# zongh5a/MDF-Net

Hardware: AMD Instinct MI355X
Metric: views/sec at DTU 1600x1200x5-view x4-scale (higher is better)
Workload: dtype f32; 1 GPU; DTU eval 1600x1184 (1600x1200 cropped as load/dtueval.py:34), 5 views, 3 cost-volume stages + x2 refine = 4 output scales, hypotheses (48,24,8), batch 1 per rank, seeded random weights (pth/dtu_29.pth is not available offline); parallelism=views sharded over 1 rank(s), no collective

## Files before the change

### mdf-net_amd/csrc/wino2d.hip

```cpp
#include <cstdlib>
#include <type_traits>
#include "common.h"
#include "conv_lds_common.h"
#define W3_PINNED_TILES_32
#include "wino3d_acc.h"

namespace {

template <int I, int N, typename F>
__device__ __forceinline__ void static_for(F&& f) {
  if constexpr (I < N) {
    f(std::integral_constant<int, I>{});
    static_for<I + 1, N>(f);
  }
}

struct Wino2dParams {
  const float* x;
  const float* wpack;
  const float* alpha;
  const float* beta;
  const float* res;
  float* y;
  float res_scale;
  int B, H, W, relu;
  int tiles_h, tiles_w, n_tiles;
};

template <int CIN, int COUT>
struct W2 {
  static_assert(CIN % 16 == 0 && COUT % 16 == 0 && COUT <= 64 && CIN <= 128, "2-D Winograd form: Cin, Cout multiples of 16, Cout <= 64");
  static constexpr int PASSES = (CIN > 64) ? 2 : 1, CP = CIN / PASSES;
  static constexpr int NCH = CP / 16, NT = COUT / 16, NG = CP / 4;
  static constexpr int WN = (CP >= 64) ? 2 : 1, NTW = NT / WN, WM = 4 / WN;
  static_assert(NT % WN == 0 && NTW >= 1 && NTW <= 2, "cout tiles per wave");
  static constexpr int TH = 2 * WM, TWO = 32;
  static constexpr int PH = TH + 2, PW = TWO + 2;
  static constexpr int NPP = PH * PW;
  static constexpr int S = round_s(NPP, 4, 2);
  static constexpr int PLANE = CP * S;
  static constexpr int RING = 3;
  static constexpr int NPOS = NG * NPP;
  static constexpr int NFILL = (NPOS + 255) / 256;
  static constexpr int EPI_OFF = RING * PLANE;
  static constexpr int FRAG = 64 * 4;
  static constexpr int NSTEP = NCH * 16;
  static constexpr bool WL = ((size_t)(RING * PLANE + 128 + PASSES * NSTEP * NT * FRAG) * sizeof(float) <= 160 * 1024);
  static constexpr int W_OFF = EPI_OFF + 128;
  static constexpr size_t LDS_BYTES = (size_t)(RING * PLANE + 128 + (WL ? PASSES * NSTEP * NT * FRAG : 0)) * sizeof(float);
  static_assert(S > NPP, "a pad vector per group takes the fill's surplus lanes");
};

template <int CIN, bool S2D, bool SKIP, int PAD = 0>
struct W2Live {
  static constexpr int CM = CIN / 4, NSTEP = CIN;
  static constexpr bool all_odd(int ch, int bit) {
    for (int c = ch * 16; c < ch * 16 + 16; ++c)
      if (!(((c / CM) >> bit) & 1)) return false;
    return true;
  }
  static constexpr bool py1(int ch) { return S2D && SKIP && all_odd(ch, 1); }
  static constexpr bool px1(int ch) { return S2D && SKIP && all_odd(ch, 0); }
  static constexpr bool zero(int ch, int ab) { return (py1(ch) && (ab >> 2) == 3) || (px1(ch) && (ab & 3) == 3); }
  static constexpr bool kept(int ch, int ab) {
    if (!zero(ch, ab)) return false;
    int n = 0;
    for (int i = 0; i < ch * 16 + ab; ++i) n += zero(i / 16, i % 16) ? 1 : 0;
    return n < PAD;
  }
  static constexpr bool dead(int ch, int ab) { return zero(ch, ab) && !kept(ch, ab); }
  static constexpr bool kept_ok() {
    for (int i = 0; i < NSTEP; ++i)
      if (kept(i / 16, i % 16) && (i % 16 == 0 || zero(i / 16, i % 16 - 1))) return false;
    return true;
  }
  static constexpr bool need(int ch, int e) { return !(py1(ch) && (e >> 2) == 3) && !(px1(ch) && (e & 3) == 3); }
  static constexpr int count(int upto = NSTEP) {
    int n = 0;
    for (int i = 0; i < upto; ++i) n += dead(i / 16, i % 16) ? 0 : 1;
    return n;
  }
  static constexpr int nth(int j) {
    for (int i = 0; i < NSTEP; ++i)
      if (!dead(i / 16, i % 16) && j-- == 0) return i;
    return -1;
  }
  static constexpr bool chunk0_live() {
    for (int ab = 0; ab < 16; ++ab)
      if (dead(0, ab)) return false;
    return true;
  }
};

#ifndef MDF_W2_DIAG
#define MDF_W2_DIAG 0
#endif
#ifndef MDF_W2_HOLD_REL
#define MDF_W2_HOLD_REL 0
#endif
#ifndef MDF_W2_NA
#define MDF_W2_NA 4
#endif
#ifndef MDF_W2_WRITE_AB
#define MDF_W2_WRITE_AB 2
#endif

template <int CIN, int COUT, int NA, int WRITE_AB, bool S2D, bool SKIP = true, int PAD = 0>
__global__ __launch_bounds__(256, 1) void wino2d_kernel(const Wino2dParams p) {
  typedef W2<CIN, COUT> C;
  typedef W2Live<CIN, S2D, SKIP, PAD> LV;
  constexpr int NCH = C::NCH, NT = C::NT, S = C::S, PW = C::PW, NPP = C::NPP, NFILL = C::NFILL, NSTEP = C::NSTEP, PASSES = C::PASSES;
  constexpr int AH = NA - 1;
  constexpr int NL = LV::count();
  static_assert(PASSES * NSTEP == LV::NSTEP && (PASSES == 1 || S2D), "passes: the parity form only");
  static_assert(NA >= 2 && NL % NA == 0, "the fragment ring must close over a tile");
  static_assert(LV::chunk0_live(), "every accumulator tile's first step is in chunk 0 of pass 0 (mfma_fresh)");
  static_assert(LV::kept_ok(), "a kept zero step has a computed V[ab - 1]");
  extern __shared__ __attribute__((aligned(16))) float lds[];

  const int tid = threadIdx.x, lane = tid & 63;
  const int wave = __builtin_amdgcn_readfirstlane(tid >> 6);
  const int q = lane >> 4, n16 = lane & 15;
  const __amdgpu_buffer_rsrc_t wres = make_rsrc(p.wpack, (unsigned)(PASSES * NSTEP * NT * 64 * 4 * 4));
  const int wvoff = lane * 16;
  const int wm = wave / C::WN, wn = wave % C::WN;
  constexpr int NTW = C::NTW;
  const int lane_lds = (q * S + wm * 2 * PW + n16 * 2) * 4;

  if (tid < 128) {
    const int c = tid & 63;
    lds[C::EPI_OFF + tid] = (tid < 64) ? ((c < COUT && p.alpha) ? p.alpha[c] : 1.f) : ((c < COUT && p.beta) ? p.beta[c] : 0.f);
  }
  if constexpr (C::WL) {
    constexpr int NV = PASSES * NSTEP * NT * 64;
    for (int v = tid; v < NV; v += 256)
      *reinterpret_cast<float4*>(lds + C::W_OFF + v * 4) = *reinterpret_cast<const float4*>(p.wpack + (size_t)v * 4);
  }

  constexpr bool HOLD_REL = (NFILL <= 11) || (NTW == 1) || MDF_W2_HOLD_REL;
  constexpr int CM = S2D ? CIN / 4 : CIN;
  [[maybe_unused]] constexpr int GPP = CM / 4;
  static_assert(HOLD_REL ? PASSES == 1 : true, "held offsets are those of pass 0");
  auto rel_of = [&](int row, int col, int g, int pass) -> int {
    if constexpr (S2D) {
      const int gl = pass * C::NG + g, par = gl / GPP, c4 = gl - par * GPP;
      return (((2 * row + (par >> 1)) * (2 * p.W) + 2 * col + (par & 1)) * CM + c4 * 4) * 4;
    } else {
      return ((row * p.W + col) * CIN + g * 4) * 4;
    }
  };
  int f_lds[NFILL], f_rc[NFILL], f_rel[HOLD_REL ? NFILL : 1];
#pragma unroll
  for (int k = 0; k < NFILL; ++k) {
    const int idx = tid + k * 256;
    const int glo = idx & 3, r = idx >> 2;
    const int v = r % NPP, g = (r / NPP) * 4 + glo;
    const bool live = idx < C::NPOS;
    const int row = live ? v / PW : 0x40, col = v % PW;
    f_lds[k] = live ? (g * S + v) * 4 : NPP * 4;
    f_rc[k] = (row << 16) | (col << 8) | g;
    if constexpr (HOLD_REL) f_rel[k] = live ? rel_of(row, col, g, 0) : (int)0x80000000u;
  }

  const unsigned lb = mdf::xcd_remap(blockIdx.x, gridDim.x);
  const int t_begin = __builtin_amdgcn_readfirstlane((int)((unsigned long long)lb * (unsigned)p.n_tiles / gridDim.x));
  const int t_end = __builtin_amdgcn_readfirstlane((int)((unsigned long long)(lb + 1) * (unsigned)p.n_tiles / gridDim.x));
  if (t_begin >= t_end) return;

  float4 pf[NFILL];
  struct TileAt { int b, th, tw; };
  auto tile_at = [&](int t) -> TileAt {
    const int tw = t % p.tiles_w, rest = t / p.tiles_w;
    return TileAt{__builtin_amdgcn_readfirstlane(rest / p.tiles_h), __builtin_amdgcn_readfirstlane(rest % p.tiles_h), __builtin_amdgcn_readfirstlane(tw)};
  };
  auto tile_advance = [&](TileAt& c) {
    if (++c.tw == p.tiles_w) {
      c.tw = 0;
      if (++c.th == p.tiles_h) { c.th = 0; ++c.b; }
    }
  };
  auto issue_tile = [&](const TileAt& at, int pass, bool valid) {
    const int b = valid ? at.b : 0, h0 = (valid ? at.th : 0) * C::TH, w0 = (valid ? at.tw : 0) * C::TWO;
    const long long org = S2D ? ((long long)b * (2 * p.H) + 2 * (h0 - 1)) * (2 * p.W) + 2 * (w0 - 1)
                              : ((long long)b * p.H + (h0 - 1)) * p.W + (w0 - 1);
    const float* pz = p.x + org * CM;
    const unsigned long long pa = (unsigned long long)pz;
    const unsigned lo = (unsigned)__builtin_amdgcn_readfirstlane((int)(unsigned)pa), hi = (unsigned)__builtin_amdgcn_readfirstlane((int)(unsigned)(pa >> 32));
    const unsigned nrec = (!valid || (MDF_W2_DIAG & 1)) ? 0u : 0x7fffffffu;
    const __amdgpu_buffer_rsrc_t xr = make_rsrc((const void*)(((unsigned long long)hi << 32) | lo), nrec);
    const int r_lo = 1 - h0, r_hi = p.H + 1 - h0, c_lo = 1 - w0, c_hi = p.W + 1 - w0;
    if constexpr (HOLD_REL) {
      if (r_lo <= 0 && r_hi >= C::PH && c_lo <= 0 && c_hi >= C::PW) {
#pragma unroll
        for (int k = 0; k < NFILL; ++k) {
          const u32x4_t v = __builtin_amdgcn_raw_buffer_load_b128(xr, f_rel[k], 0, 0);
          pf[k] = make_float4(__uint_as_float(v.x), __uint_as_float(v.y), __uint_as_float(v.z), __uint_as_float(v.w));
        }
        return;
      }
    }
#pragma unroll
    for (int k = 0; k < NFILL; ++k) {
      const int row = f_rc[k] >> 16, col = (f_rc[k] >> 8) & 0xff;
      const bool ok = row >= r_lo && row < r_hi && col >= c_lo && col < c_hi;
      int rel;
      if constexpr (HOLD_REL) rel = f_rel[k];
      else rel = rel_of(row, col, f_rc[k] & 0xff, pass);
      const u32x4_t v = __builtin_amdgcn_raw_buffer_load_b128(xr, ok ? rel : (int)0x80000000u, 0, 0);
      pf[k] = make_float4(__uint_as_float(v.x), __uint_as_float(v.y), __uint_as_float(v.z), __uint_as_float(v.w));
    }
  };
  auto write_tile = [&](int slot) {
#pragma unroll
    for (int k = 0; k < NFILL; ++k) *reinterpret_cast<float4*>(lds + slot * C::PLANE + f_lds[k]) = pf[k];
  };

  f32x2_t V[16][2], Dn[16][2];
  auto read_elem = [&](int slot, int ch, int e) {
    const int i = e >> 2, j = e & 3;
    float t[4];
    lds_frag<4>(lds + slot * C::PLANE + lane_lds + ((ch * 4) * S + i * PW + j) * 4, t);
    Dn[e][0] = (f32x2_t){t[0], t[1]};
    Dn[e][1] = (f32x2_t){t[2], t[3]};
  };
  auto transform = [&](auto lcc) {
    constexpr int LC = decltype(lcc)::value;
    constexpr bool PY = LV::py1(LC), PX = LV::px1(LC);
#pragma unroll
    for (int j = 0; j < (PX ? 3 : 4); ++j)
#pragma unroll
      for (int c = 0; c < 2; ++c) {
        const f32x2_t d0 = Dn[j][c], d1 = Dn[4 + j][c], d2 = Dn[8 + j][c];
        Dn[j][c] = d0 - d2; Dn[4 + j][c] = d1 + d2; Dn[8 + j][c] = d2 - d1;
        if constexpr (!PY) { const f32x2_t d3 = Dn[12 + j][c]; Dn[12 + j][c] = d1 - d3; }
      }
#pragma unroll
    for (int a = 0; a < (PY ? 3 : 4); ++a)
#pragma unroll
      for (int c = 0; c < 2; ++c) {
        const f32x2_t e0 = Dn[a * 4][c], e1 = Dn[a * 4 + 1][c], e2 = Dn[a * 4 + 2][c];
        V[a * 4][c] = e0 - e2; V[a * 4 + 1][c] = e1 + e2; V[a * 4 + 2][c] = e2 - e1;
        if constexpr (!PX) { const f32x2_t e3 = Dn[a * 4 + 3][c]; V[a * 4 + 3][c] = e1 - e3; }
      }
#pragma unroll
    for (int e = 0; e < 16; ++e) {
      if ((PY && (e >> 2) == 3) || (PX && (e & 3) == 3)) continue;
#pragma unroll
      for (int c = 0; c < 2; ++c) asm volatile("" : "+v"(V[e][c]));
    }
  };

  float af[NA][NTW][4];
  auto load_a = [&](int i, int buf) {
#pragma unroll
    for (int ntl = 0; ntl < NTW; ++ntl) {
      if constexpr (C::WL) lds_frag<4>(lds + C::W_OFF + (i * NT + wn * NTW + ntl) * C::FRAG + lane * 4, af[buf][ntl]);
      else buf_load_to<4>(wres, wvoff, (i * NT + wn * NTW + ntl) * (64 * 4 * 4), af[buf][ntl]);
    }
  };

  auto epilogue = [&](const TileAt& at) {
    const int b = at.b, h0 = at.th * C::TH, w0 = at.tw * C::TWO;
    if (h0 + 2 * wm >= p.H) return;
    const float* epi_tab = lds + C::EPI_OFF;
    asm volatile("s_nop 15\n\ts_nop 15" ::: "memory");
    static_for<0, NTW>([&](auto ntc) {
      constexpr int nt = decltype(ntc)::value;
      const int c0 = (wn * NTW + nt) * 16 + 4 * q;
      float yv[2][2][4];
      static_for<0, 2>([&](auto k2c) {
        constexpr int k2 = decltype(k2c)::value;
        float m[16][2];
        static_for<0, 16>([&](auto abc) { AccTile<nt * 16 + decltype(abc)::value>::template read2<k2>(m[decltype(abc)::value]); });
        f32x2_t srow[2][4];
#pragma unroll
        for (int bb = 0; bb < 4; ++bb) {
          const f32x2_t m0 = {m[bb][0], m[bb][1]}, m1 = {m[4 + bb][0], m[4 + bb][1]};
          const f32x2_t m2 = {m[8 + bb][0], m[8 + bb][1]}, m3 = {m[12 + bb][0], m[12 + bb][1]};
          srow[0][bb] = m0 + m1 + m2;
          srow[1][bb] = m1 - m2 - m3;
        }
#pragma unroll
        for (int pr = 0; pr < 2; ++pr) {
          const f32x2_t y0 = srow[pr][0] + srow[pr][1] + srow[pr][2];
          const f32x2_t y1 = srow[pr][1] - srow[pr][2] - srow[pr][3];
          yv[pr][0][2 * k2] = y0[0]; yv[pr][0][2 * k2 + 1] = y0[1];
          yv[pr][1][2 * k2] = y1[0]; yv[pr][1][2 * k2 + 1] = y1[1];
        }
      });
      float al_l[4], be_l[4];
#pragma unroll
      for (int k = 0; k < 4; ++k) { al_l[k] = epi_tab[c0 + k]; be_l[k] = epi_tab[64 + c0 + k]; }
#pragma unroll
      for (int pr = 0; pr < 2; ++pr) {
        const int h = h0 + 2 * wm + pr;
        if (h >= p.H) continue;
        const size_t row_vox = ((size_t)b * p.H + h) * p.W;
#pragma unroll
        for (int rr = 0; rr < 2; ++rr) {
          const int ow = w0 + 2 * n16 + rr;
          if (ow >= p.W) continue;
          float ov[4];
#pragma unroll
          for (int k = 0; k < 4; ++k) {
            ov[k] = yv[pr][rr][k] * al_l[k] + be_l[k];
            if (p.relu) ov[k] = fmaxf(ov[k], 0.f);
          }
          const size_t oi = (row_vox + ow) * COUT + c0;
          if (p.res) {
            const float4 rv = *reinterpret_cast<const float4*>(p.res + oi);
            ov[0] = rv.x + ov[0] * p.res_scale; ov[1] = rv.y + ov[1] * p.res_scale;
            ov[2] = rv.z + ov[2] * p.res_scale; ov[3] = rv.w + ov[3] * p.res_scale;
          }
          if (!(MDF_W2_DIAG & 2) || ov[0] == 1234.5f) *reinterpret_cast<float4*>(p.y + oi) = make_float4(ov[0], ov[1], ov[2], ov[3]);
        }
      }
    });
  };

  auto step = [&](auto rc, auto pc, const TileAt& at, const TileAt& at_n, bool valid_n, bool has_next) {
    constexpr int R = decltype(rc)::value, P = decltype(pc)::value;
    constexpr int SLOT_N = (R + 1) % 3;
    constexpr int LC_NEXT = (P + 1 < PASSES) ? (P + 1) * NCH : 0;
    static_for<0, NSTEP>([&](auto ic) {
      constexpr int i = decltype(ic)::value;
      constexpr int ch = i / 16, ab = i % 16;
      constexpr int lc = P * NCH + ch, li = P * NSTEP + i;
      constexpr bool last_chunk = (ch == NCH - 1);
      constexpr bool live = !LV::dead(lc, ab);
      [[maybe_unused]] constexpr int j = LV::count(li);
      if constexpr (live) {
        constexpr int ahead = LV::nth((j + AH) % NL);
        if (!(MDF_W2_DIAG & 16)) load_a(ahead, (j + AH) % NA);
      }
      if constexpr (ch == 0 && ab == WRITE_AB) {
        if (has_next) {
          write_tile(SLOT_N);
          __syncthreads();
        }
      }
      if constexpr (ab > WRITE_AB && ab <= WRITE_AB + 8 && !(MDF_W2_DIAG & 32)) {
        constexpr int e0 = 2 * (ab - WRITE_AB - 1);
        constexpr int lcn = last_chunk ? LC_NEXT : lc + 1;
        static_for<0, 2>([&](auto kc) {
          constexpr int e = e0 + decltype(kc)::value;
          if constexpr (LV::need(lcn, e)) {
            if constexpr (!last_chunk) read_elem(R, ch + 1, e);
            else read_elem(SLOT_N, 0, e);
          }
        });
      }
      __builtin_amdgcn_sched_barrier(0);
      if constexpr (live) {
        static_for<0, NTW>([&](auto ntc) {
          constexpr int nt = decltype(ntc)::value;
          constexpr int T = nt * 16 + ab;
          constexpr int vb = LV::kept(lc, ab) ? ab - 1 : ab;
          if constexpr (lc == 0) AccTile<T>::mfma_fresh(af[j % NA][nt][0], V[vb][0][0]);
          else AccTile<T>::mfma(af[j % NA][nt][0], V[vb][0][0]);
          AccTile<T>::mfma(af[j % NA][nt][1], V[vb][0][1]);
          AccTile<T>::mfma(af[j % NA][nt][2], V[vb][1][0]);
          AccTile<T>::mfma(af[j % NA][nt][3], V[vb][1][1]);
        });
      }
      __builtin_amdgcn_sched_barrier(0);
      if constexpr (ab == 15 && !last_chunk) { if (!(MDF_W2_DIAG & 8)) transform(std::integral_constant<int, lc + 1>{}); }
    });
    issue_tile(at_n, P, valid_n);
    if (!(MDF_W2_DIAG & 8)) transform(std::integral_constant<int, LC_NEXT>{});
    if constexpr (P == PASSES - 1) { if (!(MDF_W2_DIAG & 4)) epilogue(at); }
  };

  int t = t_begin;
  const int t_last = t_end - 1;
  TileAt at = tile_at(t), at2 = at;
  issue_tile(at, 0, true);
  write_tile(0);
  __syncthreads();
  tile_advance(at2);
  if constexpr (PASSES == 1) {
    issue_tile(at2, 0, t < t_last);
    tile_advance(at2);
  } else {
    issue_tile(at, 1, true);
  }
#pragma unroll
  for (int e = 0; e < 16; ++e) read_elem(0, 0, e);
  transform(std::integral_constant<int, 0>{});
  static_for<0, AH>([&](auto ic) {
    constexpr int first = LV::nth(decltype(ic)::value);
    load_a(first, decltype(ic)::value % NA);
  });

#define W2_STEP(RR, PP)                                                                                                          \
  {                                                                                                                              \
    const bool more = t < t_last;                                                                                                \
    if constexpr (PASSES == 1) step(std::integral_constant<int, RR>{}, std::integral_constant<int, 0>{}, at, at2, t + 2 <= t_last, more); \
    else step(std::integral_constant<int, RR>{}, std::integral_constant<int, PP>{}, at, at2, more, (PP) == 0 || more);           \
    if constexpr ((PP) == PASSES - 1) {                                                                                          \
      if (!more) break;                                                                                                          \
      ++t; tile_advance(at); tile_advance(at2);                                                                                  \
    }                                                                                                                            \
  }
  if constexpr (PASSES == 1) {
    for (;;) {
      W2_STEP(0, 0)
      W2_STEP(1, 0)
      W2_STEP(2, 0)
    }
  } else {
    for (;;) {
      W2_STEP(0, 0)
      W2_STEP(1, 1)
      W2_STEP(2, 0)
      W2_STEP(0, 1)
      W2_STEP(1, 0)
      W2_STEP(2, 1)
    }
  }
#undef W2_STEP
}

template <int CIN, int COUT, bool S2D = false, bool SKIP = true, int NA = MDF_W2_NA, int PAD = 0>
int launch_wino2d(Wino2dParams& p, hipStream_t st) {
  typedef W2<CIN, COUT> C;
  constexpr int WRITE_AB = MDF_W2_WRITE_AB;
  p.tiles_h = (p.H + C::TH - 1) / C::TH;
  p.tiles_w = (p.W + C::TWO - 1) / C::TWO;
  const long long tiles = (long long)p.B * p.tiles_h * p.tiles_w;
  if (tiles >= (1ll << 31)) return MDF_EUNSUPPORTED;
  p.n_tiles = (int)tiles;
  constexpr auto kern = &wino2d_kernel<CIN, COUT, NA, WRITE_AB, S2D, S2D && SKIP, PAD>;
  if (int rc = mdf::ensure_dynamic_lds<kern>(C::LDS_BYTES)) return rc;
  long long grid = 256;
  grid = mdf::env_pos("MDF_WINO2D_GRID", grid);
  if (grid > tiles / 2) grid = tiles / 2;
  if (grid < 1) grid = 1;
  hipLaunchKernelGGL(kern, dim3((unsigned)grid), dim3(256), C::LDS_BYTES, st, p);
  return mdf::check_launch("wino2d_kernel");
}

}

int mdf_wino2d_dispatch(const float* x, const float* wpack_wino, const float* alpha, const float* beta, const float* res, float res_scale,
                        float* y, int B, int H, int W, int Cin, int Cout, int relu, void* stream) {
  Wino2dParams p{};
  p.x = x; p.wpack = wpack_wino; p.alpha = alpha; p.beta = beta; p.res = res; p.res_scale = res_scale; p.y = y;
  p.B = B; p.H = H; p.W = W; p.relu = relu;
  if ((long long)B * H * W * Cin * 4 >= (1ll << 31)) return MDF_EUNSUPPORTED;
  if (Cin == 16 && Cout == 16 && getenv("MDF_WINO2D_16")) return launch_wino2d<16, 16>(p, (hipStream_t)stream);
  if (Cin == 32 && Cout == 32) return launch_wino2d<32, 32>(p, (hipStream_t)stream);
  if (Cin == 64 && Cout == 64) return launch_wino2d<64, 64>(p, (hipStream_t)stream);
  return MDF_EUNSUPPORTED;
}

int mdf_wino2d_s2d_dispatch(const float* x, const float* wpack_k5w, const float* alpha, const float* beta, float* y, int B, int Ho, int Wo,
                            int Cin_mem, int Cout, int relu, void* stream) {
  Wino2dParams p{};
  p.x = x; p.wpack = wpack_k5w; p.alpha = alpha; p.beta = beta; p.res = nullptr; p.res_scale = 0.f; p.y = y;
  p.B = B; p.H = Ho; p.W = Wo; p.relu = relu;
  if ((long long)B * Ho * Wo * 4 * Cin_mem * 4 >= (1ll << 31)) return MDF_EUNSUPPORTED;
  const bool skip = mdf::env_flag("MDF_WINO2D_SKIP", true);
  hipStream_t st = (hipStream_t)stream;
  if (Cin_mem == 32 && Cout == 64) return skip ? launch_wino2d<128, 64, true, true, 4, 2>(p, st) : launch_wino2d<128, 64, true, false>(p, st);
  if (Cin_mem == 16 && Cout == 32) return skip ? launch_wino2d<64, 32, true, true, 7, 0>(p, st) : launch_wino2d<64, 32, true, false>(p, st);
  if (Cin_mem == 8 && Cout == 16) return launch_wino2d<32, 16, true, false>(p, st);
  return MDF_EUNSUPPORTED;
}
```

Before: 308.1 views/s.

## Cover ragged right edge of 2-D Winograd conv with narrow tall strip tiles

When the image width leaves a small remainder past the last full 32-wide tile column, the kernel now handles that remainder with 16x8 strip tiles instead of a full 8x32 tile that is mostly padding. The tile loop is wrapped in a templated run lambda, instantiated once for ordinary tiles and once for strips, and each block processes its ordinary range then its strip range. This cuts wasted MFMA and fill work on the mostly-empty edge tiles. The cost is a second code instantiation, which raises code size and register pressure, plus an extra barrier between the two phases. Strips can be turned off with an environment variable.

```diff
diff --git a/mdf-net_amd/csrc/wino2d.hip b/mdf-net_amd/csrc/wino2d.hip
--- a/mdf-net_amd/csrc/wino2d.hip
+++ b/mdf-net_amd/csrc/wino2d.hip
@@ -24,7 +24,10 @@
   float* y;
   float res_scale;
   int B, H, W, relu;
-  int tiles_h, tiles_w, n_tiles;
+  int tiles_h, tiles_w;
+  int strips_h;
+  int n_ord;
+  int n_tiles;
 };
 
 template <int CIN, int COUT>
@@ -37,6 +40,9 @@
   static constexpr int TH = 2 * WM, TWO = 32;
   static constexpr int PH = TH + 2, PW = TWO + 2;
   static constexpr int NPP = PH * PW;
+  static constexpr bool STRIPS = (WM == 2);
+  static constexpr int STH = 16, STW = 8, SPH = STH + 2, SPW = STW + 2;
+  static_assert(!STRIPS || (SPH * SPW <= NPP && STH == 8 * WM && TWO % STW == 0), "strip tiles: the patch fits the plane, 4 row pairs x 4 column pairs per wave");
   static constexpr int S = round_s(NPP, 4, 2);
   static constexpr int PLANE = CP * S;
   static constexpr int RING = 3;
@@ -109,7 +115,7 @@
 __global__ __launch_bounds__(256, 1) void wino2d_kernel(const Wino2dParams p) {
   typedef W2<CIN, COUT> C;
   typedef W2Live<CIN, S2D, SKIP, PAD> LV;
-  constexpr int NCH = C::NCH, NT = C::NT, S = C::S, PW = C::PW, NPP = C::NPP, NFILL = C::NFILL, NSTEP = C::NSTEP, PASSES = C::PASSES;
+  constexpr int NCH = C::NCH, NT = C::NT, S = C::S, NSTEP = C::NSTEP, PASSES = C::PASSES;
   constexpr int AH = NA - 1;
   constexpr int NL = LV::count();
   static_assert(PASSES * NSTEP == LV::NSTEP && (PASSES == 1 || S2D), "passes: the parity form only");
@@ -120,12 +126,10 @@
 
   const int tid = threadIdx.x, lane = tid & 63;
   const int wave = __builtin_amdgcn_readfirstlane(tid >> 6);
-  const int q = lane >> 4, n16 = lane & 15;
   const __amdgpu_buffer_rsrc_t wres = make_rsrc(p.wpack, (unsigned)(PASSES * NSTEP * NT * 64 * 4 * 4));
   const int wvoff = lane * 16;
   const int wm = wave / C::WN, wn = wave % C::WN;
   constexpr int NTW = C::NTW;
-  const int lane_lds = (q * S + wm * 2 * PW + n16 * 2) * 4;
 
   if (tid < 128) {
     const int c = tid & 63;
@@ -137,288 +141,322 @@
       *reinterpret_cast<float4*>(lds + C::W_OFF + v * 4) = *reinterpret_cast<const float4*>(p.wpack + (size_t)v * 4);
   }
 
-  constexpr bool HOLD_REL = (NFILL <= 11) || (NTW == 1) || MDF_W2_HOLD_REL;
-  constexpr int CM = S2D ? CIN / 4 : CIN;
-  [[maybe_unused]] constexpr int GPP = CM / 4;
-  static_assert(HOLD_REL ? PASSES == 1 : true, "held offsets are those of pass 0");
-  auto rel_of = [&](int row, int col, int g, int pass) -> int {
-    if constexpr (S2D) {
-      const int gl = pass * C::NG + g, par = gl / GPP, c4 = gl - par * GPP;
-      return (((2 * row + (par >> 1)) * (2 * p.W) + 2 * col + (par & 1)) * CM + c4 * 4) * 4;
-    } else {
-      return ((row * p.W + col) * CIN + g * 4) * 4;
-    }
-  };
-  int f_lds[NFILL], f_rc[NFILL], f_rel[HOLD_REL ? NFILL : 1];
-#pragma unroll
-  for (int k = 0; k < NFILL; ++k) {
-    const int idx = tid + k * 256;
-    const int glo = idx & 3, r = idx >> 2;
-    const int v = r % NPP, g = (r / NPP) * 4 + glo;
-    const bool live = idx < C::NPOS;
-    const int row = live ? v / PW : 0x40, col = v % PW;
-    f_lds[k] = live ? (g * S + v) * 4 : NPP * 4;
-    f_rc[k] = (row << 16) | (col << 8) | g;
-    if constexpr (HOLD_REL) f_rel[k] = live ? rel_of(row, col, g, 0) : (int)0x80000000u;
-  }
-
   const unsigned lb = mdf::xcd_remap(blockIdx.x, gridDim.x);
   const int t_begin = __builtin_amdgcn_readfirstlane((int)((unsigned long long)lb * (unsigned)p.n_tiles / gridDim.x));
   const int t_end = __builtin_amdgcn_readfirstlane((int)((unsigned long long)(lb + 1) * (unsigned)p.n_tiles / gridDim.x));
   if (t_begin >= t_end) return;
 
-  float4 pf[NFILL];
-  struct TileAt { int b, th, tw; };
-  auto tile_at = [&](int t) -> TileAt {
-    const int tw = t % p.tiles_w, rest = t / p.tiles_w;
-    return TileAt{__builtin_amdgcn_readfirstlane(rest / p.tiles_h), __builtin_amdgcn_readfirstlane(rest % p.tiles_h), __builtin_amdgcn_readfirstlane(tw)};
-  };
-  auto tile_advance = [&](TileAt& c) {
-    if (++c.tw == p.tiles_w) {
-      c.tw = 0;
-      if (++c.th == p.tiles_h) { c.th = 0; ++c.b; }
+  auto run = [&](auto kindc, const int t_b, const int t_e, [[maybe_unused]] const int n_ord, [[maybe_unused]] const int strips_h) {
+    constexpr bool STRIP = decltype(kindc)::value == 1;
+    constexpr int TH = STRIP ? C::STH : C::TH, PH = STRIP ? C::SPH : C::PH, PW = STRIP ? C::SPW : C::PW;
+    constexpr int NPP = PH * PW, NPOS = C::NG * NPP, NFILL = (NPOS + 255) / 256;
+    int tid_l = tid;
+    asm volatile("" : "+v"(tid_l));
+    const int q = (tid_l & 63) >> 4, n16 = tid_l & 15;
+    const int rp = STRIP ? 4 * wm + (n16 & 3) : wm, cp = STRIP ? (n16 >> 2) : n16;
+    const int lane_lds = (q * S + rp * 2 * PW + cp * 2) * 4;
+
+    constexpr bool HOLD_REL = (C::NFILL <= 11) || (NTW == 1) || MDF_W2_HOLD_REL;
+    constexpr int CM = S2D ? CIN / 4 : CIN;
+    [[maybe_unused]] constexpr int GPP = CM / 4;
+    static_assert(HOLD_REL ? PASSES == 1 : true, "held offsets are those of pass 0");
+    auto rel_of = [&](int row, int col, int g, int pass) -> int {
+      if constexpr (S2D) {
+        const int gl = pass * C::NG + g, par = gl / GPP, c4 = gl - par * GPP;
+        return (((2 * row + (par >> 1)) * (2 * p.W) + 2 * col + (par & 1)) * CM + c4 * 4) * 4;
+      } else {
+        return ((row * p.W + col) * CIN + g * 4) * 4;
+      }
+    };
+    int f_lds[NFILL], f_rc[NFILL], f_rel[HOLD_REL ? NFILL : 1];
+#pragma unroll
+    for (int k = 0; k < NFILL; ++k) {
+      const int idx = tid_l + k * 256;
+      const int glo = idx & 3, r = idx >> 2;
+      const int v = r % NPP, g = (r / NPP) * 4 + glo;
+      const bool live = idx < NPOS;
+      const int row = live ? v / PW : 0x40, col = v % PW;
+      f_lds[k] = live ? (g * S + v) * 4 : C::NPP * 4;
+      f_rc[k] = (row << 16) | (col << 8) | g;
+      if constexpr (HOLD_REL) f_rel[k] = live ? rel_of(row, col, g, 0) : (int)0x80000000u;
     }
-  };
-  auto issue_tile = [&](const TileAt& at, int pass, bool valid) {
-    const int b = valid ? at.b : 0, h0 = (valid ? at.th : 0) * C::TH, w0 = (valid ? at.tw : 0) * C::TWO;
-    const long long org = S2D ? ((long long)b * (2 * p.H) + 2 * (h0 - 1)) * (2 * p.W) + 2 * (w0 - 1)
-                              : ((long long)b * p.H + (h0 - 1)) * p.W + (w0 - 1);
-    const float* pz = p.x + org * CM;
-    const unsigned long long pa = (unsigned long long)pz;
-    const unsigned lo = (unsigned)__builtin_amdgcn_readfirstlane((int)(unsigned)pa), hi = (unsigned)__builtin_amdgcn_readfirstlane((int)(unsigned)(pa >> 32));
-    const unsigned nrec = (!valid || (MDF_W2_DIAG & 1)) ? 0u : 0x7fffffffu;
-    const __amdgpu_buffer_rsrc_t xr = make_rsrc((const void*)(((unsigned long long)hi << 32) | lo), nrec);
-    const int r_lo = 1 - h0, r_hi = p.H + 1 - h0, c_lo = 1 - w0, c_hi = p.W + 1 - w0;
-    if constexpr (HOLD_REL) {
-      if (r_lo <= 0 && r_hi >= C::PH && c_lo <= 0 && c_hi >= C::PW) {
-#pragma unroll
-        for (int k = 0; k < NFILL; ++k) {
-          const u32x4_t v = __builtin_amdgcn_raw_buffer_load_b128(xr, f_rel[k], 0, 0);
-          pf[k] = make_float4(__uint_as_float(v.x), __uint_as_float(v.y), __uint_as_float(v.z), __uint_as_float(v.w));
-        }
-        return;
-      }
-    }
-#pragma unroll
-    for (int k = 0; k < NFILL; ++k) {
-      const int row = f_rc[k] >> 16, col = (f_rc[k] >> 8) & 0xff;
-      const bool ok = row >= r_lo && row < r_hi && col >= c_lo && col < c_hi;
-      int rel;
-      if constexpr (HOLD_REL) rel = f_rel[k];
-      else rel = rel_of(row, col, f_rc[k] & 0xff, pass);
-      const u32x4_t v = __builtin_amdgcn_raw_buffer_load_b128(xr, ok ? rel : (int)0x80000000u, 0, 0);
-      pf[k] = make_float4(__uint_as_float(v.x), __uint_as_float(v.y), __uint_as_float(v.z), __uint_as_float(v.w));
-    }
-  };
-  auto write_tile = [&](int slot) {
-#pragma unroll
-    for (int k = 0; k < NFILL; ++k) *reinterpret_cast<float4*>(lds + slot * C::PLANE + f_lds[k]) = pf[k];
-  };
-
-  f32x2_t V[16][2], Dn[16][2];
-  auto read_elem = [&](int slot, int ch, int e) {
-    const int i = e >> 2, j = e & 3;
-    float t[4];
-    lds_frag<4>(lds + slot * C::PLANE + lane_lds + ((ch * 4) * S + i * PW + j) * 4, t);
-    Dn[e][0] = (f32x2_t){t[0], t[1]};
-    Dn[e][1] = (f32x2_t){t[2], t[3]};
-  };
-  auto transform = [&](auto lcc) {
-    constexpr int LC = decltype(lcc)::value;
-    constexpr bool PY = LV::py1(LC), PX = LV::px1(LC);
-#pragma unroll
-    for (int j = 0; j < (PX ? 3 : 4); ++j)
-#pragma unroll
-      for (int c = 0; c < 2; ++c) {
-        const f32x2_t d0 = Dn[j][c], d1 = Dn[4 + j][c], d2 = Dn[8 + j][c];
-        Dn[j][c] = d0 - d2; Dn[4 + j][c] = d1 + d2; Dn[8 + j][c] = d2 - d1;
-        if constexpr (!PY) { const f32x2_t d3 = Dn[12 + j][c]; Dn[12 + j][c] = d1 - d3; }
-      }
-#pragma unroll
-    for (int a = 0; a < (PY ? 3 : 4); ++a)
-#pragma unroll
-      for (int c = 0; c < 2; ++c) {
-        const f32x2_t e0 = Dn[a * 4][c], e1 = Dn[a * 4 + 1][c], e2 = Dn[a * 4 + 2][c];
-        V[a * 4][c] = e0 - e2; V[a * 4 + 1][c] = e1 + e2; V[a * 4 + 2][c] = e2 - e1;
-        if constexpr (!PX) { const f32x2_t e3 = Dn[a * 4 + 3][c]; V[a * 4 + 3][c] = e1 - e3; }
-      }
-#pragma unroll
-    for (int e = 0; e < 16; ++e) {
-      if ((PY && (e >> 2) == 3) || (PX && (e & 3) == 3)) continue;
-#pragma unroll
-      for (int c = 0; c < 2; ++c) asm volatile("" : "+v"(V[e][c]));
-    }
-  };
-
-  float af[NA][NTW][4];
-  auto load_a = [&](int i, int buf) {
-#pragma unroll
-    for (int ntl = 0; ntl < NTW; ++ntl) {
-      if constexpr (C::WL) lds_frag<4>(lds + C::W_OFF + (i * NT + wn * NTW + ntl) * C::FRAG + lane * 4, af[buf][ntl]);
-      else buf_load_to<4>(wres, wvoff, (i * NT + wn * NTW + ntl) * (64 * 4 * 4), af[buf][ntl]);
-    }
-  };
-
-  auto epilogue = [&](const TileAt& at) {
-    const int b = at.b, h0 = at.th * C::TH, w0 = at.tw * C::TWO;
-    if (h0 + 2 * wm >= p.H) return;
-    const float* epi_tab = lds + C::EPI_OFF;
-    asm volatile("s_nop 15\n\ts_nop 15" ::: "memory");
-    static_for<0, NTW>([&](auto ntc) {
-      constexpr int nt = decltype(ntc)::value;
-      const int c0 = (wn * NTW + nt) * 16 + 4 * q;
-      float yv[2][2][4];
-      static_for<0, 2>([&](auto k2c) {
-        constexpr int k2 = decltype(k2c)::value;
-        float m[16][2];
-        static_for<0, 16>([&](auto abc) { AccTile<nt * 16 + decltype(abc)::value>::template read2<k2>(m[decltype(abc)::value]); });
-        f32x2_t srow[2][4];
-#pragma unroll
-        for (int bb = 0; bb < 4; ++bb) {
-          const f32x2_t m0 = {m[bb][0], m[bb][1]}, m1 = {m[4 + bb][0], m[4 + bb][1]};
-          const f32x2_t m2 = {m[8 + bb][0], m[8 + bb][1]}, m3 = {m[12 + bb][0], m[12 + bb][1]};
-          srow[0][bb] = m0 + m1 + m2;
-          srow[1][bb] = m1 - m2 - m3;
-        }
-#pragma unroll
-        for (int pr = 0; pr < 2; ++pr) {
-          const f32x2_t y0 = srow[pr][0] + srow[pr][1] + srow[pr][2];
-          const f32x2_t y1 = srow[pr][1] - srow[pr][2] - srow[pr][3];
-          yv[pr][0][2 * k2] = y0[0]; yv[pr][0][2 * k2 + 1] = y0[1];
-          yv[pr][1][2 * k2] = y1[0]; yv[pr][1][2 * k2 + 1] = y1[1];
-        }
-      });
-      float al_l[4], be_l[4];
-#pragma unroll
-      for (int k = 0; k < 4; ++k) { al_l[k] = epi_tab[c0 + k]; be_l[k] = epi_tab[64 + c0 + k]; }
-#pragma unroll
-      for (int pr = 0; pr < 2; ++pr) {
-        const int h = h0 + 2 * wm + pr;
-        if (h >= p.H) continue;
-        const size_t row_vox = ((size_t)b * p.H + h) * p.W;
-#pragma unroll
-        for (int rr = 0; rr < 2; ++rr) {
-          const int ow = w0 + 2 * n16 + rr;
-          if (ow >= p.W) continue;
-          float ov[4];
-#pragma unroll
-          for (int k = 0; k < 4; ++k) {
-            ov[k] = yv[pr][rr][k] * al_l[k] + be_l[k];
-            if (p.relu) ov[k] = fmaxf(ov[k], 0.f);
+
+    float4 pf[NFILL];
+    struct TileAt { int b, th, tw; };
+    auto tile_at = [&](int t) -> TileAt {
+      if constexpr (STRIP) {
+        const int sl = t - n_ord;
+        return TileAt{__builtin_amdgcn_readfirstlane(sl / strips_h), __builtin_amdgcn_readfirstlane(sl % strips_h), p.tiles_w};
+      } else {
+        const int tw = t % p.tiles_w, rest = t / p.tiles_w;
+        return TileAt{__builtin_amdgcn_readfirstlane(rest / p.tiles_h), __builtin_amdgcn_readfirstlane(rest % p.tiles_h), __builtin_amdgcn_readfirstlane(tw)};
+      }
+    };
+    auto tile_advance = [&](TileAt& c) {
+      if constexpr (STRIP) {
+        if (++c.th == strips_h) { c.th = 0; ++c.b; }
+      } else {
+        if (++c.tw == p.tiles_w) {
+          c.tw = 0;
+          if (++c.th == p.tiles_h) { c.th = 0; ++c.b; }
+        }
+      }
+    };
+    auto issue_tile = [&](const TileAt& at, int pass, bool valid) {
+      const int b = valid ? at.b : 0, h0 = (valid ? at.th : 0) * TH, w0 = (valid ? at.tw : 0) * C::TWO;
+      const long long org = S2D ? ((long long)b * (2 * p.H) + 2 * (h0 - 1)) * (2 * p.W) + 2 * (w0 - 1)
+                                : ((long long)b * p.H + (h0 - 1)) * p.W + (w0 - 1);
+      const float* pz = p.x + org * CM;
+      const unsigned long long pa = (unsigned long long)pz;
+      const unsigned lo = (unsigned)__builtin_amdgcn_readfirstlane((int)(unsigned)pa), hi = (unsigned)__builtin_amdgcn_readfirstlane((int)(unsigned)(pa >> 32));
+      const unsigned nrec = (!valid || (MDF_W2_DIAG & 1)) ? 0u : 0x7fffffffu;
+      const __amdgpu_buffer_rsrc_t xr = make_rsrc((const void*)(((unsigned long long)hi << 32) | lo), nrec);
+      const int r_lo = 1 - h0, r_hi = p.H + 1 - h0, c_lo = 1 - w0, c_hi = p.W + 1 - w0;
+      if constexpr (HOLD_REL && !STRIP) {
+        if (r_lo <= 0 && r_hi >= PH && c_lo <= 0 && c_hi >= PW) {
+#pragma unroll
+          for (int k = 0; k < NFILL; ++k) {
+            const u32x4_t v = __builtin_amdgcn_raw_buffer_load_b128(xr, f_rel[k], 0, 0);
+            pf[k] = make_float4(__uint_as_float(v.x), __uint_as_float(v.y), __uint_as_float(v.z), __uint_as_float(v.w));
           }
-          const size_t oi = (row_vox + ow) * COUT + c0;
-          if (p.res) {
-            const float4 rv = *reinterpret_cast<const float4*>(p.res + oi);
-            ov[0] = rv.x + ov[0] * p.res_scale; ov[1] = rv.y + ov[1] * p.res_scale;
-            ov[2] = rv.z + ov[2] * p.res_scale; ov[3] = rv.w + ov[3] * p.res_scale;
+          return;
+        }
+      }
+#pragma unroll
+      for (int k = 0; k < NFILL; ++k) {
+        const int row = f_rc[k] >> 16, col = (f_rc[k] >> 8) & 0xff;
+        const bool ok = row >= r_lo && row < r_hi && col >= c_lo && col < c_hi;
+        int rel;
+        if constexpr (HOLD_REL) rel = f_rel[k];
+        else rel = rel_of(row, col, f_rc[k] & 0xff, pass);
+        const u32x4_t v = __builtin_amdgcn_raw_buffer_load_b128(xr, ok ? rel : (int)0x80000000u, 0, 0);
+        pf[k] = make_float4(__uint_as_float(v.x), __uint_as_float(v.y), __uint_as_float(v.z), __uint_as_float(v.w));
+      }
+    };
+    auto write_tile = [&](int slot) {
+#pragma unroll
+      for (int k = 0; k < NFILL; ++k) *reinterpret_cast<float4*>(lds + slot * C::PLANE + f_lds[k]) = pf[k];
+    };
+
+    f32x2_t V[16][2], Dn[16][2];
+    auto read_elem = [&](int slot, int ch, int e) {
+      const int i = e >> 2, j = e & 3;
+      float t[4];
+      lds_frag<4>(lds + slot * C::PLANE + lane_lds + ((ch * 4) * S + i * PW + j) * 4, t);
+      Dn[e][0] = (f32x2_t){t[0], t[1]};
+      Dn[e][1] = (f32x2_t){t[2], t[3]};
+    };
+    auto transform = [&](auto lcc) {
+      constexpr int LC = decltype(lcc)::value;
+      constexpr bool PY = LV::py1(LC), PX = LV::px1(LC);
+#pragma unroll
+      for (int j = 0; j < (PX ? 3 : 4); ++j)
+#pragma unroll
+        for (int c = 0; c < 2; ++c) {
+          const f32x2_t d0 = Dn[j][c], d1 = Dn[4 + j][c], d2 = Dn[8 + j][c];
+          Dn[j][c] = d0 - d2; Dn[4 + j][c] = d1 + d2; Dn[8 + j][c] = d2 - d1;
+          if constexpr (!PY) { const f32x2_t d3 = Dn[12 + j][c]; Dn[12 + j][c] = d1 - d3; }
+        }
+#pragma unroll
+      for (int a = 0; a < (PY ? 3 : 4); ++a)
+#pragma unroll
+        for (int c = 0; c < 2; ++c) {
+          const f32x2_t e0 = Dn[a * 4][c], e1 = Dn[a * 4 + 1][c], e2 = Dn[a * 4 + 2][c];
+          V[a * 4][c] = e0 - e2; V[a * 4 + 1][c] = e1 + e2; V[a * 4 + 2][c] = e2 - e1;
+          if constexpr (!PX) { const f32x2_t e3 = Dn[a * 4 + 3][c]; V[a * 4 + 3][c] = e1 - e3; }
+        }
+#pragma unroll
+      for (int e = 0; e < 16; ++e) {
+        if ((PY && (e >> 2) == 3) || (PX && (e & 3) == 3)) continue;
+#pragma unroll
+        for (int c = 0; c < 2; ++c) asm volatile("" : "+v"(V[e][c]));
+      }
+    };
+
+    float af[NA][NTW][4];
+    auto load_a = [&](int i, int buf) {
+#pragma unroll
+      for (int ntl = 0; ntl < NTW; ++ntl) {
+        if constexpr (C::WL) lds_frag<4>(lds + C::W_OFF + (i * NT + wn * NTW + ntl) * C::FRAG + lane * 4, af[buf][ntl]);
+        else buf_load_to<4>(wres, wvoff, (i * NT + wn * NTW + ntl) * (64 * 4 * 4), af[buf][ntl]);
+      }
+    };
+
+    auto epilogue = [&](const TileAt& at) {
+      const int b = at.b, h0 = at.th * TH, w0 = at.tw * C::TWO;
+      if (h0 + 2 * (STRIP ? 4 * wm : wm) >= p.H) return;
+      const float* epi_tab = lds + C::EPI_OFF;
+      asm volatile("s_nop 15\n\ts_nop 15" ::: "memory");
+      static_for<0, NTW>([&](auto ntc) {
+        constexpr int nt = decltype(ntc)::value;
+        const int c0 = (wn * NTW + nt) * 16 + 4 * q;
+        float yv[2][2][4];
+        static_for<0, 2>([&](auto k2c) {
+          constexpr int k2 = decltype(k2c)::value;
+          float m[16][2];
+          static_for<0, 16>([&](auto abc) { AccTile<nt * 16 + decltype(abc)::value>::template read2<k2>(m[decltype(abc)::value]); });
+          f32x2_t srow[2][4];
+#pragma unroll
+          for (int bb = 0; bb < 4; ++bb) {
+            const f32x2_t m0 = {m[bb][0], m[bb][1]}, m1 = {m[4 + bb][0], m[4 + bb][1]};
+            const f32x2_t m2 = {m[8 + bb][0], m[8 + bb][1]}, m3 = {m[12 + bb][0], m[12 + bb][1]};
+            srow[0][bb] = m0 + m1 + m2;
+            srow[1][bb] = m1 - m2 - m3;
           }
-          if (!(MDF_W2_DIAG & 2) || ov[0] == 1234.5f) *reinterpret_cast<float4*>(p.y + oi) = make_float4(ov[0], ov[1], ov[2], ov[3]);
-        }
-      }
-    });
-  };
-
-  auto step = [&](auto rc, auto pc, const TileAt& at, const TileAt& at_n, bool valid_n, bool has_next) {
-    constexpr int R = decltype(rc)::value, P = decltype(pc)::value;
-    constexpr int SLOT_N = (R + 1) % 3;
-    constexpr int LC_NEXT = (P + 1 < PASSES) ? (P + 1) * NCH : 0;
-    static_for<0, NSTEP>([&](auto ic) {
-      constexpr int i = decltype(ic)::value;
-      constexpr int ch = i / 16, ab = i % 16;
-      constexpr int lc = P * NCH + ch, li = P * NSTEP + i;
-      constexpr bool last_chunk = (ch == NCH - 1);
-      constexpr bool live = !LV::dead(lc, ab);
-      [[maybe_unused]] constexpr int j = LV::count(li);
-      if constexpr (live) {
-        constexpr int ahead = LV::nth((j + AH) % NL);
-        if (!(MDF_W2_DIAG & 16)) load_a(ahead, (j + AH) % NA);
-      }
-      if constexpr (ch == 0 && ab == WRITE_AB) {
-        if (has_next) {
-          write_tile(SLOT_N);
-          __syncthreads();
-        }
-      }
-      if constexpr (ab > WRITE_AB && ab <= WRITE_AB + 8 && !(MDF_W2_DIAG & 32)) {
-        constexpr int e0 = 2 * (ab - WRITE_AB - 1);
-        constexpr int lcn = last_chunk ? LC_NEXT : lc + 1;
-        static_for<0, 2>([&](auto kc) {
-          constexpr int e = e0 + decltype(kc)::value;
-          if constexpr (LV::need(lcn, e)) {
-            if constexpr (!last_chunk) read_elem(R, ch + 1, e);
-            else read_elem(SLOT_N, 0, e);
+#pragma unroll
+          for (int pr = 0; pr < 2; ++pr) {
+            const f32x2_t y0 = srow[pr][0] + srow[pr][1] + srow[pr][2];
+            const f32x2_t y1 = srow[pr][1] - srow[pr][2] - srow[pr][3];
+            yv[pr][0][2 * k2] = y0[0]; yv[pr][0][2 * k2 + 1] = y0[1];
+            yv[pr][1][2 * k2] = y1[0]; yv[pr][1][2 * k2 + 1] = y1[1];
           }
         });
-      }
-      __builtin_amdgcn_sched_barrier(0);
-      if constexpr (live) {
-        static_for<0, NTW>([&](auto ntc) {
-          constexpr int nt = decltype(ntc)::value;
-          constexpr int T = nt * 16 + ab;
-          constexpr int vb = LV::kept(lc, ab) ? ab - 1 : ab;
-          if constexpr (lc == 0) AccTile<T>::mfma_fresh(af[j % NA][nt][0], V[vb][0][0]);
-          else AccTile<T>::mfma(af[j % NA][nt][0], V[vb][0][0]);
-          AccTile<T>::mfma(af[j % NA][nt][1], V[vb][0][1]);
-          AccTile<T>::mfma(af[j % NA][nt][2], V[vb][1][0]);
-          AccTile<T>::mfma(af[j % NA][nt][3], V[vb][1][1]);
-        });
-      }
-      __builtin_amdgcn_sched_barrier(0);
-      if constexpr (ab == 15 && !last_chunk) { if (!(MDF_W2_DIAG & 8)) transform(std::integral_constant<int, lc + 1>{}); }
+        float al_l[4], be_l[4];
+#pragma unroll
+        for (int k = 0; k < 4; ++k) { al_l[k] = epi_tab[c0 + k]; be_l[k] = epi_tab[64 + c0 + k]; }
+#pragma unroll
+        for (int pr = 0; pr < 2; ++pr) {
+          const int h = h0 + 2 * rp + pr;
+          if (h >= p.H) continue;
+          const size_t row_vox = ((size_t)b * p.H + h) * p.W;
+#pragma unroll
+          for (int rr = 0; rr < 2; ++rr) {
+            const int ow = w0 + 2 * cp + rr;
+            if (ow >= p.W) continue;
+            float ov[4];
+#pragma unroll
+            for (int k = 0; k < 4; ++k) {
+              ov[k] = yv[pr][rr][k] * al_l[k] + be_l[k];
+              if (p.relu) ov[k] = fmaxf(ov[k], 0.f);
+            }
+            const size_t oi = (row_vox + ow) * COUT + c0;
+            if (p.res) {
+              const float4 rv = *reinterpret_cast<const float4*>(p.res + oi);
+              ov[0] = rv.x + ov[0] * p.res_scale; ov[1] = rv.y + ov[1] * p.res_scale;
+              ov[2] = rv.z + ov[2] * p.res_scale; ov[3] = rv.w + ov[3] * p.res_scale;
+            }
+            if (!(MDF_W2_DIAG & 2) || ov[0] == 1234.5f) *reinterpret_cast<float4*>(p.y + oi) = make_float4(ov[0], ov[1], ov[2], ov[3]);
+          }
+        }
+      });
+    };
+
+    auto step = [&](auto rc, auto pc, const TileAt& at, const TileAt& at_n, bool valid_n, bool has_next) {
+      constexpr int R = decltype(rc)::value, P = decltype(pc)::value;
+      constexpr int SLOT_N = (R + 1) % 3;
+      constexpr int LC_NEXT = (P + 1 < PASSES) ? (P + 1) * NCH : 0;
+      static_for<0, NSTEP>([&](auto ic) {
+        constexpr int i = decltype(ic)::value;
+        constexpr int ch = i / 16, ab = i % 16;
+        constexpr int lc = P * NCH + ch, li = P * NSTEP + i;
+        constexpr bool last_chunk = (ch == NCH - 1);
+        constexpr bool live = !LV::dead(lc, ab);
+        [[maybe_unused]] constexpr int j = LV::count(li);
+        if constexpr (live) {
+          constexpr int ahead = LV::nth((j + AH) % NL);
+          if (!(MDF_W2_DIAG & 16)) load_a(ahead, (j + AH) % NA);
+        }
+        if constexpr (ch == 0 && ab == WRITE_AB) {
+          if (has_next) {
+            write_tile(SLOT_N);
+            __syncthreads();
+          }
+        }
+        if constexpr (ab > WRITE_AB && ab <= WRITE_AB + 8 && !(MDF_W2_DIAG & 32)) {
+          constexpr int e0 = 2 * (ab - WRITE_AB - 1);
+          constexpr int lcn = last_chunk ? LC_NEXT : lc + 1;
+          static_for<0, 2>([&](auto kc) {
+            constexpr int e = e0 + decltype(kc)::value;
+            if constexpr (LV::need(lcn, e)) {
+              if constexpr (!last_chunk) read_elem(R, ch + 1, e);
+              else read_elem(SLOT_N, 0, e);
+            }
+          });
+        }
+        __builtin_amdgcn_sched_barrier(0);
+        if constexpr (live) {
+          static_for<0, NTW>([&](auto ntc) {
+            constexpr int nt = decltype(ntc)::value;
+            constexpr int T = nt * 16 + ab;
+            constexpr int vb = LV::kept(lc, ab) ? ab - 1 : ab;
+            if constexpr (lc == 0) AccTile<T>::mfma_fresh(af[j % NA][nt][0], V[vb][0][0]);
+            else AccTile<T>::mfma(af[j % NA][nt][0], V[vb][0][0]);
+            AccTile<T>::mfma(af[j % NA][nt][1], V[vb][0][1]);
+            AccTile<T>::mfma(af[j % NA][nt][2], V[vb][1][0]);
+            AccTile<T>::mfma(af[j % NA][nt][3], V[vb][1][1]);
+          });
+        }
+        __builtin_amdgcn_sched_barrier(0);
+        if constexpr (ab == 15 && !last_chunk) { if (!(MDF_W2_DIAG & 8)) transform(std::integral_constant<int, lc + 1>{}); }
+      });
+      issue_tile(at_n, P, valid_n);
+      if (!(MDF_W2_DIAG & 8)) transform(std::integral_constant<int, LC_NEXT>{});
+      if constexpr (P == PASSES - 1) { if (!(MDF_W2_DIAG & 4)) epilogue(at); }
+    };
+
+    int t = t_b;
+    const int t_last = t_e - 1;
+    TileAt at = tile_at(t), at2 = at;
+    issue_tile(at, 0, true);
+    write_tile(0);
+    __syncthreads();
+    tile_advance(at2);
+    if constexpr (PASSES == 1) {
+      issue_tile(at2, 0, t < t_last);
+      tile_advance(at2);
+    } else {
+      issue_tile(at, 1, true);
+    }
+#pragma unroll
+    for (int e = 0; e < 16; ++e) read_elem(0, 0, e);
+    transform(std::integral_constant<int, 0>{});
+    static_for<0, AH>([&](auto ic) {
+      constexpr int first = LV::nth(decltype(ic)::value);
+      load_a(first, decltype(ic)::value % NA);
     });
-    issue_tile(at_n, P, valid_n);
-    if (!(MDF_W2_DIAG & 8)) transform(std::integral_constant<int, LC_NEXT>{});
-    if constexpr (P == PASSES - 1) { if (!(MDF_W2_DIAG & 4)) epilogue(at); }
+
+#define W2_STEP(RR, PP)                                                                                                          \
+    {                                                                                                                              \
+      const bool more = t < t_last;                                                                                                \
+      if constexpr (PASSES == 1) step(std::integral_constant<int, RR>{}, std::integral_constant<int, 0>{}, at, at2, t + 2 <= t_last, more); \
+      else step(std::integral_constant<int, RR>{}, std::integral_constant<int, PP>{}, at, at2, more, (PP) == 0 || more);           \
+      if constexpr ((PP) == PASSES - 1) {                                                                                          \
+        if (!more) break;                                                                                                          \
+        ++t; tile_advance(at); tile_advance(at2);                                                                                  \
+      }                                                                                                                            \
+    }
+    if constexpr (PASSES == 1) {
+      for (;;) {
+        W2_STEP(0, 0)
+        W2_STEP(1, 0)
+        W2_STEP(2, 0)
+      }
+    } else {
+      for (;;) {
+        W2_STEP(0, 0)
+        W2_STEP(1, 1)
+        W2_STEP(2, 0)
+        W2_STEP(0, 1)
+        W2_STEP(1, 0)
+        W2_STEP(2, 1)
+      }
+    }
+#undef W2_STEP
   };
 
-  int t = t_begin;
-  const int t_last = t_end - 1;
-  TileAt at = tile_at(t), at2 = at;
-  issue_tile(at, 0, true);
-  write_tile(0);
-  __syncthreads();
-  tile_advance(at2);
-  if constexpr (PASSES == 1) {
-    issue_tile(at2, 0, t < t_last);
-    tile_advance(at2);
-  } else {
-    issue_tile(at, 1, true);
-  }
-#pragma unroll
-  for (int e = 0; e < 16; ++e) read_elem(0, 0, e);
-  transform(std::integral_constant<int, 0>{});
-  static_for<0, AH>([&](auto ic) {
-    constexpr int first = LV::nth(decltype(ic)::value);
-    load_a(first, decltype(ic)::value % NA);
-  });
-
-#define W2_STEP(RR, PP)                                                                                                          \
-  {                                                                                                                              \
-    const bool more = t < t_last;                                                                                                \
-    if constexpr (PASSES == 1) step(std::integral_constant<int, RR>{}, std::integral_constant<int, 0>{}, at, at2, t + 2 <= t_last, more); \
-    else step(std::integral_constant<int, RR>{}, std::integral_constant<int, PP>{}, at, at2, more, (PP) == 0 || more);           \
-    if constexpr ((PP) == PASSES - 1) {                                                                                          \
-      if (!more) break;                                                                                                          \
-      ++t; tile_advance(at); tile_advance(at2);                                                                                  \
-    }                                                                                                                            \
-  }
-  if constexpr (PASSES == 1) {
-    for (;;) {
-      W2_STEP(0, 0)
-      W2_STEP(1, 0)
-      W2_STEP(2, 0)
+  if constexpr (C::STRIPS) {
+    const int t_mid = min(max(p.n_ord, t_begin), t_end);
+    int park[4] = {t_mid, t_end, p.n_ord, p.strips_h};
+    asm volatile("" : "+v"(park[0]), "+v"(park[1]), "+v"(park[2]), "+v"(park[3]));
+    if (t_begin < t_mid) run(std::integral_constant<int, 0>{}, t_begin, t_mid, 0, 0);
+    const int s_b = __builtin_amdgcn_readfirstlane(park[0]), s_e = __builtin_amdgcn_readfirstlane(park[1]);
+    if (s_b < s_e) {
+      __syncthreads();
+      run(std::integral_constant<int, 1>{}, s_b, s_e, __builtin_amdgcn_readfirstlane(park[2]), __builtin_amdgcn_readfirstlane(park[3]));
     }
   } else {
-    for (;;) {
-      W2_STEP(0, 0)
-      W2_STEP(1, 1)
-      W2_STEP(2, 0)
-      W2_STEP(0, 1)
-      W2_STEP(1, 0)
-      W2_STEP(2, 1)
-    }
-  }
-#undef W2_STEP
+    run(std::integral_constant<int, 0>{}, t_begin, t_end, 0, 0);
+  }
 }
 
 template <int CIN, int COUT, bool S2D = false, bool SKIP = true, int NA = MDF_W2_NA, int PAD = 0>
@@ -427,8 +465,18 @@
   constexpr int WRITE_AB = MDF_W2_WRITE_AB;
   p.tiles_h = (p.H + C::TH - 1) / C::TH;
   p.tiles_w = (p.W + C::TWO - 1) / C::TWO;
-  const long long tiles = (long long)p.B * p.tiles_h * p.tiles_w;
+  p.strips_h = 0;
+  if constexpr (C::STRIPS) {
+    const int w_rem = p.W % C::TWO;
+    if (w_rem >= 1 && w_rem <= C::STW && mdf::env_int("MDF_W2_STRIP", 1)) {
+      p.tiles_w = p.W / C::TWO;
+      p.strips_h = (p.H + C::STH - 1) / C::STH;
+    }
+  }
+  const long long n_ord = (long long)p.B * p.tiles_h * p.tiles_w;
+  const long long tiles = n_ord + (long long)p.B * p.strips_h;
   if (tiles >= (1ll << 31)) return MDF_EUNSUPPORTED;
+  p.n_ord = (int)n_ord;
   p.n_tiles = (int)tiles;
   constexpr auto kern = &wino2d_kernel<CIN, COUT, NA, WRITE_AB, S2D, S2D && SKIP, PAD>;
   if (int rc = mdf::ensure_dynamic_lds<kern>(C::LDS_BYTES)) return rc;
```

New measurement: 308.7 views/s (median of 6 runs). No clear change (+0.2%).
